# numz/ComfyUI-SeedVR2_VideoUpscaler

Measured on AMD Instinct MI355X. Metric: upscaled frames/sec (720p->4K, SeedVR2-3B), higher is better.
Workload: dtype bf16; 1 GPU; cfg3: SeedVR2-3B 32-frame 720p->4K clip (padded to 33 = 4n+1 for encode + DiT, 32 decoded), VAE tiled 1024/128; vae_tiled=True, parallelism=dp1, weights=random-init SeedVR2-3B + video_vae_v3 architecture (seeded)

## Files before the change

comfyui-seedvr2_videoupscaler_amd/csrc/svr_conv_sub.hip:

```cpp
#include "svr_common.h"
#include "../../include/seedvr2_hip.h"
#include <type_traits>

namespace svr {

constexpr int CS_TY = 16, CS_TX = 32, CS_HX = CS_TX + 1, CS_HY = CS_TY + 1;
constexpr int CS_NT = 256;
constexpr int CS_ROWS = CS_HX * CS_HY;
constexpr int CS_PIECES = (CS_ROWS * 4 + CS_NT - 1) / CS_NT;
constexpr int CS_ABUF = CS_PIECES * CS_NT * 16;
constexpr int CS_NBUF = 4;
constexpr int CS_EP_PITCH = 528;
constexpr int CS_EP_BYTES = 4 * 32 * CS_EP_PITCH;
constexpr int CS_LDS = CS_NBUF * CS_ABUF;
static_assert(CS_PIECES == 9 && CS_EP_BYTES <= CS_LDS, "piece schedule / epilogue parking");

template <int OFF> SVR_DEVICE void cs_rd2(bf16x8 (&r)[2], unsigned a0) {
    const unsigned a1 = a0 ^ 32u;
    asm volatile("ds_read_b128 %0, %2 offset:%4\n\tds_read_b128 %1, %3 offset:%4"
                 : "=&v"(r[0]), "=&v"(r[1]) : "v"(a0), "v"(a1), "n"(OFF) : "memory");
}
template <int N> SVR_DEVICE void cs_wait_rows(bf16x8 (&a)[2]) {
    asm volatile("s_waitcnt lgkmcnt(%2)" : "+v"(a[0]), "+v"(a[1]) : "n"(N));
    __builtin_amdgcn_sched_barrier(0);
}
template <int N> SVR_DEVICE void cs_wait_rows(bf16x8 (&a)[2], bf16x8 (&b)[2]) {
    asm volatile("s_waitcnt lgkmcnt(%4)" : "+v"(a[0]), "+v"(a[1]), "+v"(b[0]), "+v"(b[1]) : "n"(N));
    __builtin_amdgcn_sched_barrier(0);
}
template <int N> SVR_DEVICE void cs_wait_rows(bf16x8 (&a)[2], bf16x8 (&b)[2], bf16x8 (&c)[2], bf16x8 (&d)[2], bf16x8 (&e)[2]) {
    asm volatile("s_waitcnt lgkmcnt(%10)"
                 : "+v"(a[0]), "+v"(a[1]), "+v"(b[0]), "+v"(b[1]), "+v"(c[0]), "+v"(c[1]), "+v"(d[0]), "+v"(d[1]), "+v"(e[0]), "+v"(e[1])
                 : "n"(N));
    __builtin_amdgcn_sched_barrier(0);
}
template <int N> SVR_DEVICE void cs_wait_w(bf16x8 (&w)[2][2]) {
    asm volatile("s_waitcnt vmcnt(%4)" : "+v"(w[0][0]), "+v"(w[0][1]), "+v"(w[1][0]), "+v"(w[1][1]) : "n"(N));
    __builtin_amdgcn_sched_barrier(0);
}

__global__ __launch_bounds__(CS_NT, 1) void conv_sub_kernel(const svr_gemm_args a, const int band_rows) {
    constexpr int MTW = 8, NTW = 2, NT = CS_NT;
    extern __shared__ __attribute__((aligned(16))) char smem[];
    typedef __attribute__((ext_vector_type(16))) float f32x16_t;
    const svr_conv_geom& g = a.conv;
    const int tid = threadIdx.x;
    const int lane = tid & 63;
    const int wave = __builtin_amdgcn_readfirstlane(tid >> 6);
    const int wm = wave >> 1, wn = wave & 1;

    const int tiles_x = (g.W + CS_TX - 1) / CS_TX;
    const int tiles_y = (g.H + CS_TY - 1) / CS_TY;
    const int tiles_n = a.N / 128;
    int tl;
    {
        const int nwg = gridDim.x, bid = blockIdx.x;
        const int xcd = bid & 7, j = bid >> 3, q = nwg >> 3, r = nwg & 7;
        tl = (xcd < r ? xcd * (q + 1) : r * (q + 1) + (xcd - r) * q) + j;
    }
    const bool quad = a.phase.enabled && a.phase.quad != 0;
    int qp = 0;
    if (quad) { qp = tl & 3; tl >>= 2; }
    const int ph_py = quad ? (qp >> 1) : a.phase.py, ph_px = quad ? (qp & 1) : a.phase.px;
    const int pad_h = quad ? 1 - ph_py : g.ph, pad_w = quad ? 1 - ph_px : g.pw;
    const void* const w_frag = quad ? a.phase.W_frag4[qp] : a.W_frag;
    const float* const bias_p = quad ? a.phase.bias4[qp] : a.bias;
    const float* const bias_border_p = quad ? a.phase.bias_border4[qp] : a.phase.bias_border;
    const int tn = tl % tiles_n;
    int rr = tl / tiles_n;
    const int tx = rr % tiles_x; rr /= tiles_x;
    int ty, to;
    if (band_rows > 0 && band_rows < tiles_y) {
        const int per_band = band_rows * g.To;
        const int b = rr / per_band;
        const int rows_b = min(band_rows, tiles_y - b * band_rows);
        const int r2 = rr - b * per_band;
        to = r2 / rows_b;
        ty = b * band_rows + (r2 - to * rows_b);
    } else {
        ty = rr % tiles_y;
        to = rr / tiles_y;
    }
    const int y0 = ty * CS_TY, x0 = tx * CS_TX, n0 = tn * 128;

    const int cpk = g.Cin / 32;
    const int nA = g.kt * cpk;
    const int P = nA * 4;
    const int64_t frame_bytes = (int64_t)g.H * g.W * g.Cin * 2;
    const int srow = tid >> 2, spos = tid & 3;
    uint32_t poff[CS_PIECES];
    uint32_t akeys = 0;
#pragma unroll
    for (int q = 0; q < CS_PIECES; ++q) {
        const int row = q * (NT / 4) + srow;
        const int hy = row / CS_HX, hx = row - hy * CS_HX;
        const int y = y0 - pad_h + hy, x = x0 - pad_w + hx;
        const bool ok = (row < CS_ROWS) & ((unsigned)y < (unsigned)g.H) & ((unsigned)x < (unsigned)g.W);
        poff[q] = ok ? (uint32_t)(y * g.W + x) : 0xffffffffu;
        akeys |= (uint32_t)(spos ^ ((hx >> 2) & 3)) << (2 * q);
    }
    char* const wave_dst = smem + wave * 1024;
    auto frame_ptr = [&](int s) -> const char* {
        if (s >= nA) return nullptr;
        const int dt = s / cpk;
        const int c0 = (s - dt * cpk) * 32;
        int f = to + dt - g.pt;
        const char* basep = (const char*)a.A;
        if (f < 0) {
            if (g.halo != nullptr) { basep = (const char*)g.halo; f += g.halo_frames; }
            else f = 0;
        }
        return basep + (int64_t)f * frame_bytes + c0 * 2;
    };
    auto stage = [&](auto qc, const char* fptr, int buf) {
        constexpr int Q = decltype(qc)::value;
        const int ck = (akeys >> (2 * Q)) & 3;
        const char* src = (poff[Q] == 0xffffffffu || fptr == nullptr) ? (const char*)g.zeros
                                                                      : fptr + ((int64_t)poff[Q] * g.Cin + ck * 8) * 2;
        glds16(src, wave_dst + buf * CS_ABUF + Q * (NT * 16));
    };
    auto stage_all = [&](const char* fptr, int buf) {
        stage(std::integral_constant<int, 0>{}, fptr, buf); stage(std::integral_constant<int, 1>{}, fptr, buf);
        stage(std::integral_constant<int, 2>{}, fptr, buf); stage(std::integral_constant<int, 3>{}, fptr, buf);
        stage(std::integral_constant<int, 4>{}, fptr, buf); stage(std::integral_constant<int, 5>{}, fptr, buf);
        stage(std::integral_constant<int, 6>{}, fptr, buf); stage(std::integral_constant<int, 7>{}, fptr, buf);
        stage(std::integral_constant<int, 8>{}, fptr, buf);
    };

    const int l31 = lane & 31, hi = lane >> 5;
    const unsigned lds0 = (unsigned)(uintptr_t)(__attribute__((address_space(3))) char*)smem;
    unsigned fa[2];
#pragma unroll
    for (int dx = 0; dx < 2; ++dx)
        fa[dx] = lds0 + (unsigned)((wm * MTW * CS_HX + l31) * 64 + ((hi ^ (((dx + l31) >> 2) & 3)) << 4));

    f32x16_t acc[MTW][NTW];
#pragma unroll
    for (int y = 0; y < MTW; ++y)
#pragma unroll
        for (int z = 0; z < NTW; ++z)
#pragma unroll
            for (int e = 0; e < 16; ++e) acc[y][z][e] = 0.f;
    bf16x8 a0[2], a1[2], a2[2], a3[2], a4[2], a5[2], a6[2], a7[2], a8[2];
    bf16x8 w0[NTW][2], w1[NTW][2], w2[NTW][2], w3[NTW][2];

    const int64_t nstride = (int64_t)P * 2048;
    const char* wp0 = (const char*)w_frag + (int64_t)(n0 / 32 + wn * 2) * nstride;
    const char* wp1 = wp0 + nstride;
    const int voff = lane * 16;
    auto wload = [&](bf16x8 (&w)[NTW][2], int k) {
        auto uniform_ptr = [](const char* p) {
            const uint64_t u = (uint64_t)p;
            const uint32_t lo = __builtin_amdgcn_readfirstlane((uint32_t)u), hi_ = __builtin_amdgcn_readfirstlane((uint32_t)(u >> 32));
            return (const char*)(((uint64_t)hi_ << 32) | lo);
        };
        const char* p0 = uniform_ptr(wp0 + (int64_t)min(k, P - 1) * 2048);
        const char* p1 = uniform_ptr(wp1 + (int64_t)min(k, P - 1) * 2048);
        asm volatile("global_load_dwordx4 %0, %1, %2" : "=v"(w[0][0]) : "v"(voff), "s"(p0) : "memory");
        asm volatile("global_load_dwordx4 %0, %1, %2 offset:1024" : "=v"(w[0][1]) : "v"(voff), "s"(p0) : "memory");
        asm volatile("global_load_dwordx4 %0, %1, %2" : "=v"(w[1][0]) : "v"(voff), "s"(p1) : "memory");
        asm volatile("global_load_dwordx4 %0, %1, %2 offset:1024" : "=v"(w[1][1]) : "v"(voff), "s"(p1) : "memory");
    };

#define CS_RD(ROW, R, DXV, BUFOFF) cs_rd2<((R) * CS_HX + (DXV)) * 64>(ROW, fa[DXV] + (BUFOFF))
#define CS_MM(W, KS, ROW, MT, NTI) \
    acc[MT][NTI] = __builtin_amdgcn_mfma_f32_32x32x16_bf16(W[NTI][KS], ROW[KS], acc[MT][NTI], 0, 0, 0)
#define CS_MM8(W, RA, MA, RB, MB) \
    CS_MM(W, 0, RA, MA, 0); CS_MM(W, 0, RA, MA, 1); CS_MM(W, 0, RB, MB, 0); CS_MM(W, 0, RB, MB, 1); \
    CS_MM(W, 1, RA, MA, 0); CS_MM(W, 1, RA, MA, 1); CS_MM(W, 1, RB, MB, 0); CS_MM(W, 1, RB, MB, 1)

    auto interval = [&](auto jc, int s, const char* fstage, bf16x8 (&wc)[NTW][2], bf16x8 (&wn_)[NTW][2]) {
        constexpr int J = decltype(jc)::value;
        constexpr int DX = J >> 1, DY = J & 1;
        constexpr int NPC[4] = {0, 0, 5, 4};
        constexpr int NV = 4 + NPC[(J + 3) & 3] + NPC[(J + 2) & 3];
        const int k = s * 4 + J;
        const unsigned cur = (unsigned)((s & 3) * CS_ABUF), nxt = (unsigned)(((s + 1) & 3) * CS_ABUF);
        const int sbuf = (s + 3) & 3;
        constexpr int NDX = DX ^ 1;
        const unsigned nb = DX == 0 ? cur : nxt;
        if constexpr (DY == 0) {
            CS_RD(a8, 8, DX, cur);
            cs_wait_rows<8>(a0, a1, a2, a3, a4);
            cs_wait_w<NV>(wc);
            CS_MM8(wc, a0, 0, a1, 1);
            __builtin_amdgcn_sched_barrier(0);
            CS_RD(a0, 0, NDX, nb);
            wload(wn_, k + 2);
            __builtin_amdgcn_sched_barrier(0);
            CS_MM8(wc, a2, 2, a3, 3);
            __builtin_amdgcn_sched_barrier(0);
            if constexpr (J == 2) {
                stage(std::integral_constant<int, 0>{}, fstage, sbuf); stage(std::integral_constant<int, 1>{}, fstage, sbuf);
                stage(std::integral_constant<int, 2>{}, fstage, sbuf);
            }
            cs_wait_rows<8>(a4, a5);
            CS_MM8(wc, a4, 4, a5, 5);
            __builtin_amdgcn_sched_barrier(0);
            if constexpr (J == 2) { stage(std::integral_constant<int, 3>{}, fstage, sbuf); stage(std::integral_constant<int, 4>{}, fstage, sbuf); }
            cs_wait_rows<4>(a6, a7);
            CS_MM8(wc, a6, 6, a7, 7);
            __builtin_amdgcn_sched_barrier(0);
        } else {
            cs_wait_w<NV>(wc);
            CS_MM8(wc, a1, 0, a2, 1);
            __builtin_amdgcn_sched_barrier(0);
            CS_RD(a1, 1, NDX, nb); CS_RD(a2, 2, NDX, nb);
            wload(wn_, k + 2);
            __builtin_amdgcn_sched_barrier(0);
            CS_MM8(wc, a3, 2, a4, 3);
            __builtin_amdgcn_sched_barrier(0);
            CS_RD(a3, 3, NDX, nb); CS_RD(a4, 4, NDX, nb);
            if constexpr (J == 3) { stage(std::integral_constant<int, 5>{}, fstage, sbuf); stage(std::integral_constant<int, 6>{}, fstage, sbuf); }
            __builtin_amdgcn_sched_barrier(0);
            CS_MM8(wc, a5, 4, a6, 5);
            __builtin_amdgcn_sched_barrier(0);
            CS_RD(a5, 5, NDX, nb); CS_RD(a6, 6, NDX, nb);
            if constexpr (J == 3) { stage(std::integral_constant<int, 7>{}, fstage, sbuf); stage(std::integral_constant<int, 8>{}, fstage, sbuf); }
            cs_wait_rows<14>(a8);
            CS_MM8(wc, a7, 6, a8, 7);
            __builtin_amdgcn_sched_barrier(0);
            CS_RD(a7, 7, NDX, nb);
            if constexpr (J == 1) {
                __builtin_amdgcn_s_barrier();
                __builtin_amdgcn_sched_barrier(0);
            }
        }
    };

    stage_all(frame_ptr(0), 0);
    stage_all(frame_ptr(1), 1);
    stage_all(frame_ptr(2), 2);
    wload(w0, 0);
    wload(w1, 1);
    __builtin_amdgcn_sched_barrier(0);
#pragma unroll
    for (int y = 0; y < MTW; ++y)
#pragma unroll
        for (int z = 0; z < NTW; ++z) asm volatile("" : "+a"(acc[y][z]));
    asm volatile("s_waitcnt vmcnt(0)" ::: "memory");
    __builtin_amdgcn_s_barrier();
    __builtin_amdgcn_sched_barrier(0);
    CS_RD(a0, 0, 0, 0u); CS_RD(a1, 1, 0, 0u); CS_RD(a2, 2, 0, 0u); CS_RD(a3, 3, 0, 0u);
    CS_RD(a4, 4, 0, 0u); CS_RD(a5, 5, 0, 0u); CS_RD(a6, 6, 0, 0u); CS_RD(a7, 7, 0, 0u);

    for (int s = 0; s < nA; ++s) {
        const char* fs = frame_ptr(s + 3);
        interval(std::integral_constant<int, 0>{}, s, fs, w0, w2);
        interval(std::integral_constant<int, 1>{}, s, fs, w1, w3);
        interval(std::integral_constant<int, 2>{}, s, fs, w2, w0);
        interval(std::integral_constant<int, 3>{}, s, fs, w3, w1);
    }
    asm volatile("s_waitcnt vmcnt(0) lgkmcnt(0)" ::: "memory");
    __builtin_amdgcn_sched_barrier(0);
    __syncthreads();
#undef CS_RD
#undef CS_MM
#undef CS_MM8

    const int hi4 = hi * 4;
    const int n = n0 + (tid & 15) * 8;
    f32x4 bias_lo = {0.f, 0.f, 0.f, 0.f}, bias_hi = {0.f, 0.f, 0.f, 0.f};
    if (bias_p) {
        bias_lo = *(const f32x4*)(bias_p + n);
        bias_hi = *(const f32x4*)(bias_p + n + 4);
    }
    const int py = a.phase.enabled ? ph_py : 0, px = a.phase.enabled ? ph_px : 0;
    const int up = a.phase.enabled ? 2 : 1, ts = a.phase.enabled ? a.phase.t_stride : 1;
    const int yb = py ? g.H - 1 : 0, xb = px ? g.W - 1 : 0;
    const float* btab = a.phase.enabled ? bias_border_p : nullptr;
    double gs0 = 0.0, gq0 = 0.0, gs1 = 0.0, gq1 = 0.0;
    auto ep_body = [&](auto o32c) {
    constexpr int OKIND = decltype(o32c)::value;
    constexpr bool O32 = OKIND == SVR_STORE_FP32;
#pragma unroll
    for (int pass = 0; pass < MTW / 2; ++pass) {
        __builtin_amdgcn_sched_barrier(0);
#pragma unroll
        for (int j = 0; j < 2; ++j) {
            char* row = smem + ((wm * 2 + j) * 32 + l31) * CS_EP_PITCH;
#pragma unroll
            for (int nt = 0; nt < NTW; ++nt) {
                const f32x16_t v = acc[2 * pass + j][nt];
#pragma unroll
                for (int gq = 0; gq < 4; ++gq) {
                    const f32x4 o = {v[4 * gq], v[4 * gq + 1], v[4 * gq + 2], v[4 * gq + 3]};
                    *(f32x4*)(row + (wn * 64 + nt * 32 + 8 * gq + hi4) * 4) = o;
                }
            }
        }
        lds_barrier();
#pragma unroll
        for (int half = 0; half < 2; ++half) {
            f32x4 lo[4], hi_[4];
            int64_t off[4];
            bool ok[4];
            int border[4];
#pragma unroll
            for (int it = 0; it < 4; ++it) {
                const int vox = ((half * 4 + it) * NT + tid) >> 4;
                const int r = vox >> 5;
                const int y = y0 + (r >> 1) * MTW + 2 * pass + (r & 1), x = x0 + (vox & 31);
                ok[it] = y < g.H && x < g.W;
                const int yc = min(y, g.H - 1), xc = min(x, g.W - 1);
                border[it] = (yc == yb ? 1 : 0) | (xc == xb ? 2 : 0);
                off[it] = (((int64_t)to * ts * (up * g.H) + up * yc + py) * (up * g.W) + up * xc + px) * a.N + n;
                lo[it] = *(const f32x4*)(smem + vox * CS_EP_PITCH + (tid & 15) * 32);
                hi_[it] = *(const f32x4*)(smem + vox * CS_EP_PITCH + (tid & 15) * 32 + 16);
            }
#pragma unroll
            for (int it = 0; it < 4; ++it) {
                f32x4 bl = bias_lo, bh = bias_hi;
                if (btab != nullptr && border[it] != 0) {
                    const float* bb = btab + (int64_t)(border[it] - 1) * a.N + n;
                    bl = *(const f32x4*)bb;
                    bh = *(const f32x4*)(bb + 4);
                }
                const float f[8] = {lo[it][0] + bl[0], lo[it][1] + bl[1], lo[it][2] + bl[2], lo[it][3] + bl[3],
                                    hi_[it][0] + bh[0], hi_[it][1] + bh[1], hi_[it][2] + bh[2], hi_[it][3] + bh[3]};
                float r[8];
                if constexpr (O32) {
                    if (ok[it]) {
                        float* cp = (float*)a.C + off[it];
                        *(float4*)cp = make_float4(f[0], f[1], f[2], f[3]);
                        *(float4*)(cp + 4) = make_float4(f[4], f[5], f[6], f[7]);
                    }
#pragma unroll
                    for (int e = 0; e < 8; ++e) r[e] = f[e];
                } else {
                    const uint4 pk = OKIND == SVR_STORE_H16 ? pack8h(f) : pack8(f);
                    if (ok[it]) *(uint4*)((bf16_t*)a.C + off[it]) = pk;
                    if constexpr (OKIND == SVR_STORE_H16) unpack8h(pk, r); else unpack8(pk, r);
                }
                if (a.gn_partial != nullptr && ok[it]) {
                    gn_accumulate4(gs0, gq0, r[0], r[1], r[2], r[3]);
                    gn_accumulate4(gs1, gq1, r[4], r[5], r[6], r[7]);
                }
            }
        }
        if (pass + 1 < MTW / 2) lds_barrier();
    }
    };
    if (a.out_f32 == SVR_STORE_FP32) ep_body(std::integral_constant<int, SVR_STORE_FP32>{});
    else if (a.out_f32 == SVR_STORE_H16) ep_body(std::integral_constant<int, SVR_STORE_H16>{});
    else ep_body(std::integral_constant<int, SVR_STORE_BF16>{});
    if (a.gn_partial) {
        __syncthreads();
        double4* red = (double4*)smem;
        double2* qsum = (double2*)(smem + NT * 32);
        red[tid] = make_double4(gs0, gq0, gs1, gq1);
        __syncthreads();
        if (tid < 32) {
            const int c = tid >> 1, h = tid & 1;
            double s_ = 0.0, q_ = 0.0;
            for (int j = 0; j < NT / 16; ++j) {
                const double4 v = red[(j << 4) | c];
                s_ += h ? v.z : v.x;
                q_ += h ? v.w : v.y;
            }
            qsum[tid] = make_double2(s_, q_);
        }
        __syncthreads();
        const int qpg = (a.N / a.gn_groups) >> 2;
        if (tid < 32 / qpg) {
            double s_ = 0.0, q_ = 0.0;
            for (int i = 0; i < qpg; ++i) { s_ += qsum[tid * qpg + i].x; q_ += qsum[tid * qpg + i].y; }
            const int nblk = tiles_y * tiles_x;
            const int per_frame = a.phase.enabled ? 4 * nblk : nblk;
            const int slot = (a.phase.enabled ? (py * 2 + px) * nblk : 0) + ty * tiles_x + tx;
            ((double2*)a.gn_partial)[((int64_t)to * ts * per_frame + slot) * a.gn_groups + (n0 >> 2) / qpg + tid] = make_double2(s_, q_);
        }
    }
}

int g_conv_sub = 1;

static bool conv_sub_gn_ok(const svr_gemm_args& a) {
    const int cpg = a.gn_groups > 0 ? a.N / a.gn_groups : 0;
    return cpg >= 4 && !(cpg & 3) && a.N % a.gn_groups == 0 && 128 % cpg == 0;
}

static bool conv_sub_eligible(const svr_gemm_args& a) {
    const svr_conv_geom& g = a.conv;
    const bool quad = a.phase.enabled && a.phase.quad != 0;
    bool ptrs = true;
    if (quad) {
        for (int p = 0; p < 4; ++p)
            ptrs = ptrs && a.phase.W_frag4[p] != nullptr && (!a.phase.bias4[p] || ((uintptr_t)a.phase.bias4[p] % 16) == 0) &&
                   (!a.phase.bias_border4[p] || ((uintptr_t)a.phase.bias_border4[p] % 16) == 0);
    } else {
        ptrs = a.W_frag != nullptr && (unsigned)g.ph <= 1u && (unsigned)g.pw <= 1u && (!a.bias || ((uintptr_t)a.bias % 16) == 0) &&
               (!a.phase.bias_border || ((uintptr_t)a.phase.bias_border % 16) == 0);
    }
    return g_conv_sub && g.enabled && ptrs && g.kh == 2 && g.kw == 2 && g.sh == 1 && g.sw == 1 && g.st == 1 &&
           g.Ho == g.H && g.Wo == g.W && g.Cin % 32 == 0 && g.kt >= 1 && g.kt <= 3 &&
           g.To == g.T + g.pt - g.kt + 1 && !a.ps.enabled && a.epilogue == SVR_EPI_BIAS && !a.resid && !a.gate &&
           (!a.gn_partial || conv_sub_gn_ok(a)) && (a.N % 128) == 0 && (a.phase.enabled || (a.ldc == a.N)) &&
           (int64_t)g.H * g.W * g.Cin * 2 < (int64_t)1 << 32 && ((uintptr_t)a.C % 16) == 0;
}

static int conv_sub_gn_blocks(const svr_gemm_args& a) {
    if (!conv_sub_eligible(a) || !conv_sub_gn_ok(a)) return 0;
    const int nblk = ((a.conv.H + CS_TY - 1) / CS_TY) * ((a.conv.W + CS_TX - 1) / CS_TX);
    return a.phase.enabled ? 4 * nblk : nblk;
}

static int launch_conv_sub(const svr_gemm_args& a, hipStream_t s) {
    const svr_conv_geom& g = a.conv;
    const int tiles = g.To * ((g.H + CS_TY - 1) / CS_TY) * ((g.W + CS_TX - 1) / CS_TX) * (a.N / 128) *
                      (a.phase.enabled && a.phase.quad ? 4 : 1);
    static uint64_t lds_attr_done = 0;
    {
        const int e = set_max_dynamic_lds((const void*)conv_sub_kernel, 160 * 1024, lds_attr_done);
        if (e != 0) return e;
    }
    hipLaunchKernelGGL(conv_sub_kernel, dim3(tiles), dim3(CS_NT), CS_LDS, s, a, g_conv_band);
    return (int)hipGetLastError();
}

__global__ __launch_bounds__(256) void conv_pack_frag_taps_kernel(const bf16_t* __restrict__ W, uint4* __restrict__ out, int N, int K,
                                                                  int kt, int kh, int kw, int Cin) {
    const int cpk = Cin / 32, taps = kh * kw, P = kt * cpk * taps;
    const int64_t idx = (int64_t)blockIdx.x * 256 + threadIdx.x;
    if (idx >= (int64_t)(N / 32) * P * 128) return;
    const int lane = (int)(idx & 63), ks = (int)((idx >> 6) & 1);
    const int kk = (int)((idx >> 7) % P), n32 = (int)((idx >> 7) / P);
    const int s = kk / taps, J = kk - s * taps;
    const int dt = s / cpk, cs = s - dt * cpk, dy = J % kh, dx = J / kh;
    const int nn = n32 * 32 + (lane & 31), c = cs * 32 + ks * 16 + (lane >> 5) * 8;
    out[idx] = *(const uint4*)(W + (int64_t)nn * K + ((dt * kh + dy) * kw + dx) * Cin + c);
}

}
```

Measured before the change: 3.748 frames/s.

## Switch conv_sub inner product from 32x32x16 to 16x16x32 bf16 MFMA tiles

Replaces the 32x32x16 MFMA accumulation in the subpixel conv kernel with 16x16x32 MFMA instructions issued through inline asm. It reworks the LDS activation read addressing, the weight fragment lane offsets, the accumulator layout (f32x4 tiles) and the epilogue LDS scatter to match. Each row read now uses the same base address with a +1024 offset instead of an XOR'd address. The change is aimed at throughput or latency of the smaller MFMA shape and a simpler fragment layout. The extra MFMA count, the s_nop padding before the wait, and the assumption that the pre-packed weight fragment layout matches the new indexing are the risks.

```diff
diff --git a/comfyui-seedvr2_videoupscaler_amd/csrc/svr_conv_sub.hip b/comfyui-seedvr2_videoupscaler_amd/csrc/svr_conv_sub.hip
--- a/comfyui-seedvr2_videoupscaler_amd/csrc/svr_conv_sub.hip
+++ b/comfyui-seedvr2_videoupscaler_amd/csrc/svr_conv_sub.hip
@@ -16,9 +16,15 @@
 static_assert(CS_PIECES == 9 && CS_EP_BYTES <= CS_LDS, "piece schedule / epilogue parking");
 
 template <int OFF> SVR_DEVICE void cs_rd2(bf16x8 (&r)[2], unsigned a0) {
-    const unsigned a1 = a0 ^ 32u;
-    asm volatile("ds_read_b128 %0, %2 offset:%4\n\tds_read_b128 %1, %3 offset:%4"
-                 : "=&v"(r[0]), "=&v"(r[1]) : "v"(a0), "v"(a1), "n"(OFF) : "memory");
+    asm volatile("ds_read_b128 %0, %2 offset:%3\n\tds_read_b128 %1, %2 offset:%4"
+                 : "=&v"(r[0]), "=&v"(r[1]) : "v"(a0), "n"(OFF), "n"(OFF + 1024) : "memory");
+}
+SVR_DEVICE void cs_mfma(f32x4& c, const bf16x8& w, const bf16x8& x) {
+    asm volatile("v_mfma_f32_16x16x32_bf16 %0, %1, %2, %0" : "+a"(c) : "v"(w), "v"(x));
+}
+SVR_DEVICE void cs_mm_row(f32x4 (&c)[2][4], const bf16x8 (&w)[2][2], const bf16x8 (&r)[2]) {
+    cs_mfma(c[0][0], w[0][0], r[0]); cs_mfma(c[0][1], w[0][1], r[0]); cs_mfma(c[0][2], w[1][0], r[0]); cs_mfma(c[0][3], w[1][1], r[0]);
+    cs_mfma(c[1][0], w[0][0], r[1]); cs_mfma(c[1][1], w[0][1], r[1]); cs_mfma(c[1][2], w[1][0], r[1]); cs_mfma(c[1][3], w[1][1], r[1]);
 }
 template <int N> SVR_DEVICE void cs_wait_rows(bf16x8 (&a)[2]) {
     asm volatile("s_waitcnt lgkmcnt(%2)" : "+v"(a[0]), "+v"(a[1]) : "n"(N));
@@ -42,7 +48,6 @@
 __global__ __launch_bounds__(CS_NT, 1) void conv_sub_kernel(const svr_gemm_args a, const int band_rows) {
     constexpr int MTW = 8, NTW = 2, NT = CS_NT;
     extern __shared__ __attribute__((aligned(16))) char smem[];
-    typedef __attribute__((ext_vector_type(16))) float f32x16_t;
     const svr_conv_geom& g = a.conv;
     const int tid = threadIdx.x;
     const int lane = tid & 63;
@@ -127,27 +132,27 @@
         stage(std::integral_constant<int, 8>{}, fptr, buf);
     };
 
-    const int l31 = lane & 31, hi = lane >> 5;
+    const int l15 = lane & 15, c4 = lane >> 4;
     const unsigned lds0 = (unsigned)(uintptr_t)(__attribute__((address_space(3))) char*)smem;
     unsigned fa[2];
 #pragma unroll
     for (int dx = 0; dx < 2; ++dx)
-        fa[dx] = lds0 + (unsigned)((wm * MTW * CS_HX + l31) * 64 + ((hi ^ (((dx + l31) >> 2) & 3)) << 4));
-
-    f32x16_t acc[MTW][NTW];
+        fa[dx] = lds0 + (unsigned)((wm * MTW * CS_HX + l15) * 64 + ((c4 ^ (((dx + l15) >> 2) & 3)) << 4));
+
+    f32x4 acc[MTW][2][2 * NTW];
 #pragma unroll
     for (int y = 0; y < MTW; ++y)
 #pragma unroll
-        for (int z = 0; z < NTW; ++z)
-#pragma unroll
-            for (int e = 0; e < 16; ++e) acc[y][z][e] = 0.f;
+        for (int z = 0; z < 4 * NTW; ++z)
+#pragma unroll
+            for (int e = 0; e < 4; ++e) acc[y][z >> 2][z & 3][e] = 0.f;
     bf16x8 a0[2], a1[2], a2[2], a3[2], a4[2], a5[2], a6[2], a7[2], a8[2];
     bf16x8 w0[NTW][2], w1[NTW][2], w2[NTW][2], w3[NTW][2];
 
     const int64_t nstride = (int64_t)P * 2048;
     const char* wp0 = (const char*)w_frag + (int64_t)(n0 / 32 + wn * 2) * nstride;
     const char* wp1 = wp0 + nstride;
-    const int voff = lane * 16;
+    const int voff = c4 * 512 + l15 * 16;
     auto wload = [&](bf16x8 (&w)[NTW][2], int k) {
         auto uniform_ptr = [](const char* p) {
             const uint64_t u = (uint64_t)p;
@@ -157,17 +162,13 @@
         const char* p0 = uniform_ptr(wp0 + (int64_t)min(k, P - 1) * 2048);
         const char* p1 = uniform_ptr(wp1 + (int64_t)min(k, P - 1) * 2048);
         asm volatile("global_load_dwordx4 %0, %1, %2" : "=v"(w[0][0]) : "v"(voff), "s"(p0) : "memory");
-        asm volatile("global_load_dwordx4 %0, %1, %2 offset:1024" : "=v"(w[0][1]) : "v"(voff), "s"(p0) : "memory");
+        asm volatile("global_load_dwordx4 %0, %1, %2 offset:256" : "=v"(w[0][1]) : "v"(voff), "s"(p0) : "memory");
         asm volatile("global_load_dwordx4 %0, %1, %2" : "=v"(w[1][0]) : "v"(voff), "s"(p1) : "memory");
-        asm volatile("global_load_dwordx4 %0, %1, %2 offset:1024" : "=v"(w[1][1]) : "v"(voff), "s"(p1) : "memory");
+        asm volatile("global_load_dwordx4 %0, %1, %2 offset:256" : "=v"(w[1][1]) : "v"(voff), "s"(p1) : "memory");
     };
 
 #define CS_RD(ROW, R, DXV, BUFOFF) cs_rd2<((R) * CS_HX + (DXV)) * 64>(ROW, fa[DXV] + (BUFOFF))
-#define CS_MM(W, KS, ROW, MT, NTI) \
-    acc[MT][NTI] = __builtin_amdgcn_mfma_f32_32x32x16_bf16(W[NTI][KS], ROW[KS], acc[MT][NTI], 0, 0, 0)
-#define CS_MM8(W, RA, MA, RB, MB) \
-    CS_MM(W, 0, RA, MA, 0); CS_MM(W, 0, RA, MA, 1); CS_MM(W, 0, RB, MB, 0); CS_MM(W, 0, RB, MB, 1); \
-    CS_MM(W, 1, RA, MA, 0); CS_MM(W, 1, RA, MA, 1); CS_MM(W, 1, RB, MB, 0); CS_MM(W, 1, RB, MB, 1)
+#define CS_MM8(W, RA, MA, RB, MB) cs_mm_row(acc[MA], W, RA); cs_mm_row(acc[MB], W, RB)
 
     auto interval = [&](auto jc, int s, const char* fstage, bf16x8 (&wc)[NTW][2], bf16x8 (&wn_)[NTW][2]) {
         constexpr int J = decltype(jc)::value;
@@ -237,7 +238,7 @@
 #pragma unroll
     for (int y = 0; y < MTW; ++y)
 #pragma unroll
-        for (int z = 0; z < NTW; ++z) asm volatile("" : "+a"(acc[y][z]));
+        for (int z = 0; z < 2; ++z) asm volatile("" : "+a"(acc[y][z][0]), "+a"(acc[y][z][1]), "+a"(acc[y][z][2]), "+a"(acc[y][z][3]));
     asm volatile("s_waitcnt vmcnt(0)" ::: "memory");
     __builtin_amdgcn_s_barrier();
     __builtin_amdgcn_sched_barrier(0);
@@ -251,14 +252,12 @@
         interval(std::integral_constant<int, 2>{}, s, fs, w2, w0);
         interval(std::integral_constant<int, 3>{}, s, fs, w3, w1);
     }
-    asm volatile("s_waitcnt vmcnt(0) lgkmcnt(0)" ::: "memory");
+    asm volatile("s_nop 7\n\ts_nop 7\n\ts_waitcnt vmcnt(0) lgkmcnt(0)" ::: "memory");
     __builtin_amdgcn_sched_barrier(0);
     __syncthreads();
 #undef CS_RD
-#undef CS_MM
 #undef CS_MM8
 
-    const int hi4 = hi * 4;
     const int n = n0 + (tid & 15) * 8;
     f32x4 bias_lo = {0.f, 0.f, 0.f, 0.f}, bias_hi = {0.f, 0.f, 0.f, 0.f};
     if (bias_p) {
@@ -278,15 +277,12 @@
         __builtin_amdgcn_sched_barrier(0);
 #pragma unroll
         for (int j = 0; j < 2; ++j) {
-            char* row = smem + ((wm * 2 + j) * 32 + l31) * CS_EP_PITCH;
-#pragma unroll
-            for (int nt = 0; nt < NTW; ++nt) {
-                const f32x16_t v = acc[2 * pass + j][nt];
-#pragma unroll
-                for (int gq = 0; gq < 4; ++gq) {
-                    const f32x4 o = {v[4 * gq], v[4 * gq + 1], v[4 * gq + 2], v[4 * gq + 3]};
-                    *(f32x4*)(row + (wn * 64 + nt * 32 + 8 * gq + hi4) * 4) = o;
-                }
+#pragma unroll
+            for (int vh = 0; vh < 2; ++vh) {
+                char* row = smem + ((wm * 2 + j) * 32 + vh * 16 + l15) * CS_EP_PITCH;
+#pragma unroll
+                for (int cb = 0; cb < 2 * NTW; ++cb)
+                    *(f32x4*)(row + (wn * 64 + cb * 16 + c4 * 4) * 4) = acc[2 * pass + j][vh][cb];
             }
         }
         lds_barrier();
```

Result: no change. 3.764 frames/s (median of 6 runs) (+0.4%).

## Switch conv_sub MFMA from 32x32x16 to 16x16x32 tiles via cg helpers

Applied to the files above, without the earlier changes.

Replaces the 32x32x16 bf16 MFMA accumulation with four 16x16 sub-tiles per 32x32 block, using the shared cg_rd2/cg_mm4 helpers. The LDS read addressing, weight fragment offsets and epilogue parking layout change to match the 16x16 lane mapping. The aim is higher MFMA throughput or better issue interleaving with the 16x16 instruction shape, at the cost of more MFMA instructions and a different register layout. It depends on helpers defined elsewhere and on the weight fragment packing matching the new offsets.

```diff
diff --git a/comfyui-seedvr2_videoupscaler_amd/csrc/svr_conv_sub.hip b/comfyui-seedvr2_videoupscaler_amd/csrc/svr_conv_sub.hip
--- a/comfyui-seedvr2_videoupscaler_amd/csrc/svr_conv_sub.hip
+++ b/comfyui-seedvr2_videoupscaler_amd/csrc/svr_conv_sub.hip
@@ -15,11 +15,6 @@
 constexpr int CS_LDS = CS_NBUF * CS_ABUF;
 static_assert(CS_PIECES == 9 && CS_EP_BYTES <= CS_LDS, "piece schedule / epilogue parking");
 
-template <int OFF> SVR_DEVICE void cs_rd2(bf16x8 (&r)[2], unsigned a0) {
-    const unsigned a1 = a0 ^ 32u;
-    asm volatile("ds_read_b128 %0, %2 offset:%4\n\tds_read_b128 %1, %3 offset:%4"
-                 : "=&v"(r[0]), "=&v"(r[1]) : "v"(a0), "v"(a1), "n"(OFF) : "memory");
-}
 template <int N> SVR_DEVICE void cs_wait_rows(bf16x8 (&a)[2]) {
     asm volatile("s_waitcnt lgkmcnt(%2)" : "+v"(a[0]), "+v"(a[1]) : "n"(N));
     __builtin_amdgcn_sched_barrier(0);
@@ -42,7 +37,6 @@
 __global__ __launch_bounds__(CS_NT, 1) void conv_sub_kernel(const svr_gemm_args a, const int band_rows) {
     constexpr int MTW = 8, NTW = 2, NT = CS_NT;
     extern __shared__ __attribute__((aligned(16))) char smem[];
-    typedef __attribute__((ext_vector_type(16))) float f32x16_t;
     const svr_conv_geom& g = a.conv;
     const int tid = threadIdx.x;
     const int lane = tid & 63;
@@ -127,27 +121,27 @@
         stage(std::integral_constant<int, 8>{}, fptr, buf);
     };
 
-    const int l31 = lane & 31, hi = lane >> 5;
+    const int l15 = lane & 15, c4 = lane >> 4;
     const unsigned lds0 = (unsigned)(uintptr_t)(__attribute__((address_space(3))) char*)smem;
     unsigned fa[2];
 #pragma unroll
     for (int dx = 0; dx < 2; ++dx)
-        fa[dx] = lds0 + (unsigned)((wm * MTW * CS_HX + l31) * 64 + ((hi ^ (((dx + l31) >> 2) & 3)) << 4));
-
-    f32x16_t acc[MTW][NTW];
+        fa[dx] = lds0 + (unsigned)((wm * MTW * CS_HX + l15) * 64 + ((c4 ^ (((dx + l15) >> 2) & 3)) << 4));
+
+    f32x4 acc[MTW][NTW][2][2];
 #pragma unroll
     for (int y = 0; y < MTW; ++y)
 #pragma unroll
         for (int z = 0; z < NTW; ++z)
 #pragma unroll
-            for (int e = 0; e < 16; ++e) acc[y][z][e] = 0.f;
+            for (int e = 0; e < 16; ++e) acc[y][z][e >> 3][(e >> 2) & 1][e & 3] = 0.f;
     bf16x8 a0[2], a1[2], a2[2], a3[2], a4[2], a5[2], a6[2], a7[2], a8[2];
     bf16x8 w0[NTW][2], w1[NTW][2], w2[NTW][2], w3[NTW][2];
 
     const int64_t nstride = (int64_t)P * 2048;
     const char* wp0 = (const char*)w_frag + (int64_t)(n0 / 32 + wn * 2) * nstride;
     const char* wp1 = wp0 + nstride;
-    const int voff = lane * 16;
+    const int voff = c4 * 512 + l15 * 16;
     auto wload = [&](bf16x8 (&w)[NTW][2], int k) {
         auto uniform_ptr = [](const char* p) {
             const uint64_t u = (uint64_t)p;
@@ -157,17 +151,14 @@
         const char* p0 = uniform_ptr(wp0 + (int64_t)min(k, P - 1) * 2048);
         const char* p1 = uniform_ptr(wp1 + (int64_t)min(k, P - 1) * 2048);
         asm volatile("global_load_dwordx4 %0, %1, %2" : "=v"(w[0][0]) : "v"(voff), "s"(p0) : "memory");
-        asm volatile("global_load_dwordx4 %0, %1, %2 offset:1024" : "=v"(w[0][1]) : "v"(voff), "s"(p0) : "memory");
+        asm volatile("global_load_dwordx4 %0, %1, %2 offset:256" : "=v"(w[0][1]) : "v"(voff), "s"(p0) : "memory");
         asm volatile("global_load_dwordx4 %0, %1, %2" : "=v"(w[1][0]) : "v"(voff), "s"(p1) : "memory");
-        asm volatile("global_load_dwordx4 %0, %1, %2 offset:1024" : "=v"(w[1][1]) : "v"(voff), "s"(p1) : "memory");
-    };
-
-#define CS_RD(ROW, R, DXV, BUFOFF) cs_rd2<((R) * CS_HX + (DXV)) * 64>(ROW, fa[DXV] + (BUFOFF))
-#define CS_MM(W, KS, ROW, MT, NTI) \
-    acc[MT][NTI] = __builtin_amdgcn_mfma_f32_32x32x16_bf16(W[NTI][KS], ROW[KS], acc[MT][NTI], 0, 0, 0)
+        asm volatile("global_load_dwordx4 %0, %1, %2 offset:256" : "=v"(w[1][1]) : "v"(voff), "s"(p1) : "memory");
+    };
+
+#define CS_RD(ROW, R, DXV, BUFOFF) cg_rd2<((R) * CS_HX + (DXV)) * 64>(ROW, fa[DXV] + (BUFOFF))
 #define CS_MM8(W, RA, MA, RB, MB) \
-    CS_MM(W, 0, RA, MA, 0); CS_MM(W, 0, RA, MA, 1); CS_MM(W, 0, RB, MB, 0); CS_MM(W, 0, RB, MB, 1); \
-    CS_MM(W, 1, RA, MA, 0); CS_MM(W, 1, RA, MA, 1); CS_MM(W, 1, RB, MB, 0); CS_MM(W, 1, RB, MB, 1)
+    cg_mm4(acc[MA][0], W[0], RA); cg_mm4(acc[MA][1], W[1], RA); cg_mm4(acc[MB][0], W[0], RB); cg_mm4(acc[MB][1], W[1], RB)
 
     auto interval = [&](auto jc, int s, const char* fstage, bf16x8 (&wc)[NTW][2], bf16x8 (&wn_)[NTW][2]) {
         constexpr int J = decltype(jc)::value;
@@ -237,7 +228,8 @@
 #pragma unroll
     for (int y = 0; y < MTW; ++y)
 #pragma unroll
-        for (int z = 0; z < NTW; ++z) asm volatile("" : "+a"(acc[y][z]));
+        for (int z = 0; z < NTW; ++z)
+            asm volatile("" : "+a"(acc[y][z][0][0]), "+a"(acc[y][z][0][1]), "+a"(acc[y][z][1][0]), "+a"(acc[y][z][1][1]));
     asm volatile("s_waitcnt vmcnt(0)" ::: "memory");
     __builtin_amdgcn_s_barrier();
     __builtin_amdgcn_sched_barrier(0);
@@ -255,10 +247,8 @@
     __builtin_amdgcn_sched_barrier(0);
     __syncthreads();
 #undef CS_RD
-#undef CS_MM
 #undef CS_MM8
 
-    const int hi4 = hi * 4;
     const int n = n0 + (tid & 15) * 8;
     f32x4 bias_lo = {0.f, 0.f, 0.f, 0.f}, bias_hi = {0.f, 0.f, 0.f, 0.f};
     if (bias_p) {
@@ -278,15 +268,14 @@
         __builtin_amdgcn_sched_barrier(0);
 #pragma unroll
         for (int j = 0; j < 2; ++j) {
-            char* row = smem + ((wm * 2 + j) * 32 + l31) * CS_EP_PITCH;
-#pragma unroll
-            for (int nt = 0; nt < NTW; ++nt) {
-                const f32x16_t v = acc[2 * pass + j][nt];
-#pragma unroll
-                for (int gq = 0; gq < 4; ++gq) {
-                    const f32x4 o = {v[4 * gq], v[4 * gq + 1], v[4 * gq + 2], v[4 * gq + 3]};
-                    *(f32x4*)(row + (wn * 64 + nt * 32 + 8 * gq + hi4) * 4) = o;
-                }
+#pragma unroll
+            for (int vh = 0; vh < 2; ++vh) {
+                char* row = smem + ((wm * 2 + j) * 32 + vh * 16 + l15) * CS_EP_PITCH;
+#pragma unroll
+                for (int nt = 0; nt < NTW; ++nt)
+#pragma unroll
+                    for (int ch = 0; ch < 2; ++ch)
+                        *(f32x4*)(row + (wn * 64 + nt * 32 + ch * 16 + c4 * 4) * 4) = acc[2 * pass + j][nt][vh][ch];
             }
         }
         lds_barrier();
```

Result: no change. 3.696 frames/s before, 3.713 frames/s after (median of 6 runs) (+0.4%).
